# petim0/fly_bProject

Measured on AMD Instinct MI355X. Metric: env-steps/sec (PPO rollout + update), 8192 envs per GPU, higher is better.
Workload: dtype f32 (optimizer step: fp16x2 operand split; rollout policy + critic: bf16x3 operand split; fp32 accumulate)

## Files before the change

### fly_bproject_amd/csrc/fs_common.inc

```
#ifndef FS_IN
#define FS_IN 73
#endif
#ifndef FS_RING
#define FS_RING 4
#endif
typedef short s16x4 __attribute__((ext_vector_type(4)));
constexpr int FS_PX = 96, FS_P1 = 256, FS_P2 = 128, FS_P4 = 32;
template <int PITCH>
__device__ __forceinline__ int fs_key(int r)
{
    if (PITCH % 128 == 0) return ((r & 3) << 2) | ((r >> 2) & 3);
    return (r >> 2) & 3;
}
template <int PITCH>
__device__ __forceinline__ int fs_off(int r, int c) { return r * PITCH + ((((c >> 3) ^ fs_key<PITCH>(r))) << 3) + (c & 7); }
template <int PITCH> constexpr int fs_plane() { return BM * PITCH; }

__device__ __forceinline__ void fs_mfma_v(f32x16& acc, const bf16x8& a, const bf16x8& b)
{
    asm volatile("v_mfma_f32_32x32x16_bf16 %0, %1, %2, %0" : "+v"(acc) : "v"(a), "v"(b));
}
__device__ __forceinline__ void fs_mfma_v0(f32x16& acc, const bf16x8& a, const bf16x8& b)
{
    asm volatile("v_mfma_f32_32x32x16_bf16 %0, %1, %2, 0" : "=&v"(acc) : "v"(a), "v"(b));
}
__device__ __forceinline__ void fs_mfma_vg(f32x16& acc, const bf16x8& a, const bf16x8& b)
{
    asm volatile("s_nop 3\n\tv_mfma_f32_32x32x16_bf16 %0, %1, %2, %0" : "+v"(acc) : "v"(a), "v"(b));
}
__device__ __forceinline__ void fs_mfma_vg0(f32x16& acc, const bf16x8& a, const bf16x8& b)
{
    asm volatile("s_nop 3\n\tv_mfma_f32_32x32x16_bf16 %0, %1, %2, 0" : "=&v"(acc) : "v"(a), "v"(b));
}
__device__ __forceinline__ void fs_mfma_settle(f32x16& acc) { asm volatile("s_nop 7\n\ts_nop 7\n\ts_nop 3" : "+v"(acc)); }
__device__ __forceinline__ void fs_mfma_settle(f32x16& a, f32x16& b) { asm volatile("s_nop 7\n\ts_nop 7\n\ts_nop 3" : "+v"(a), "+v"(b)); }

template <int K, int PITCH, bool SWAP, bool ZERO = true, int HEAD = B3_HEAD>
__device__ __forceinline__ void fs_gemm(const WeightHeadT<HEAD>& head, const u16* __restrict__ Wb, int tile0, const u16* act, int k0,
                                        f32x16& hi, f32x16& lo, int lane)
{
    constexpr int K16 = K / 16;
    constexpr int RING = K16 < FS_RING ? K16 : FS_RING;
    constexpr int ARING = K16 < B3_ARING ? K16 : B3_ARING;
    const int r = lane & 31;
    const int key = fs_key<PITCH>(r);
    const int sh = (k0 >> 3) + (lane >> 5);
    const u16* arow = act + r * PITCH;
    const u16* bp = Wb + (long)tile0 * K16 * 1536 + lane * 8;
    Frag3 b[RING], a[ARING];
    auto aload = [&](Frag3& f, int kb) {
        const u16* q = arow + (((sh + 2 * kb) ^ key) << 3);
#pragma unroll
        for (int p = 0; p < 3; ++p) f.p[p] = *reinterpret_cast<const float4*>(q + p * fs_plane<PITCH>());
    };
#pragma unroll
    for (int s = 0; s < RING; ++s) {
        if (s < ARING) aload(a[s], s);
#pragma unroll
        for (int p = 0; p < 3; ++p)
            b[s].p[p] = s < HEAD ? head.b[s].p[p] : *reinterpret_cast<const float4*>(bp + s * 1536 + p * 512);
    }
#pragma unroll
    for (int kb = 0; kb < K16; ++kb) {
        const int s = kb % RING, sa = kb % ARING;
        __builtin_amdgcn_sched_barrier(0);
        const bf16x8 w0 = as_bf16x8(b[s].p[0]), w1 = as_bf16x8(b[s].p[1]), w2 = as_bf16x8(b[s].p[2]);
        const bf16x8 x0 = as_bf16x8(a[sa].p[0]), x1 = as_bf16x8(a[sa].p[1]), x2 = as_bf16x8(a[sa].p[2]);
        if (ZERO && kb == 0) {
            if (!SWAP) { fs_mfma_v0(lo, w0, x2); fs_mfma_v0(hi, w0, x0); } else { fs_mfma_v0(lo, x2, w0); fs_mfma_v0(hi, x0, w0); }
        } else {
            if (!SWAP) { fs_mfma_v(lo, w0, x2); fs_mfma_v(hi, w0, x0); } else { fs_mfma_v(lo, x2, w0); fs_mfma_v(hi, x0, w0); }
        }
        if (!SWAP) { fs_mfma_v(lo, w2, x0); fs_mfma_v(lo, w1, x1); fs_mfma_v(lo, w0, x1); fs_mfma_v(lo, w1, x0); }
        else { fs_mfma_v(lo, x0, w2); fs_mfma_v(lo, x1, w1); fs_mfma_v(lo, x1, w0); fs_mfma_v(lo, x0, w1); }
        __builtin_amdgcn_sched_barrier(0);
        if (kb + RING < K16) {
#pragma unroll
            for (int p = 0; p < 3; ++p) b[s].p[p] = *reinterpret_cast<const float4*>(bp + (kb + RING) * 1536 + p * 512);
        }
        if (kb + ARING < K16) aload(a[sa], kb + ARING);
    }
    fs_mfma_settle(hi, lo);
    __builtin_amdgcn_sched_barrier(0);
}

template <int K, int PITCH, bool SWAP, bool ZERO, class E, int HOST_GAPS = 6 * (K / 16), int MODE = 0>
struct FsGemmHost {
    static constexpr bool SPLIT = MODE == 1;
    static constexpr int K16 = K / 16, GAPS = 6 * K16, HALF = K16 / 2;
    static constexpr int RING = K16 < FS_RING ? K16 : FS_RING;
    static constexpr int ARING = K16 < B3_ARING ? K16 : B3_ARING;
    static_assert(!SPLIT || K16 == 16, "the split order is written for K = 256");
    static_assert(HOST_GAPS <= GAPS && (MODE == 0 || HOST_GAPS <= 6 * HALF), "the guest must be done when the second half begins");
    static constexpr bool order_ok()
    {
        unsigned seen = 0;
        for (int i = 0; i < K16; ++i) {
            const int kb = kblock(i);
            if (kb < 0 || kb >= K16 || ((seen >> kb) & 1u)) return false;
            if (MODE == 1 && ((kb & 2) != 0) != (i >= HALF)) return false;
            seen |= 1u << kb;
        }
        return true;
    }
    Frag3 b[RING], a[ARING];
    const u16 *arow, *bp;
    int sh, key;
    f32x16 &hi, &lo;
    E& e;
    __device__ __forceinline__ FsGemmHost(f32x16& hi_, f32x16& lo_, E& e_) : hi(hi_), lo(lo_), e(e_) {}
    static constexpr int kblock(int i) { return !SPLIT ? i : (i < HALF ? 4 * (i >> 1) + (i & 1) : 4 * ((i - HALF) >> 1) + 2 + (i & 1)); }
    static_assert(order_ok(), "k-step order");
    __device__ __forceinline__ void aload(Frag3& f, int kb)
    {
        const u16* q = arow + (((sh + 2 * kb) ^ key) << 3);
#pragma unroll
        for (int p = 0; p < 3; ++p) f.p[p] = *reinterpret_cast<const float4*>(q + p * fs_plane<PITCH>());
    }
    __device__ __forceinline__ void bload(Frag3& f, int kb)
    {
#pragma unroll
        for (int p = 0; p < 3; ++p) f.p[p] = *reinterpret_cast<const float4*>(bp + kb * 1536 + p * 512);
    }
    template <int J>
    __device__ __forceinline__ void gap()
    {
        if constexpr (J < HOST_GAPS) {
            constexpr int T0 = J * E::TOTAL / HOST_GAPS, T1 = (J + 1) * E::TOTAL / HOST_GAPS;
            __builtin_amdgcn_sched_barrier(0);
            run<T0, T1>();
            __builtin_amdgcn_sched_barrier(0);
        }
    }
    template <int T, int TE>
    __device__ __forceinline__ void run()
    {
        if constexpr (T < TE) { e.q(T); run<T + 1, TE>(); }
    }
    template <int I>
    __device__ __forceinline__ void steps()
    {
        if constexpr (I < K16) {
            constexpr int s = I % RING, sa = I % ARING;
            if constexpr (MODE != 0 && I == HALF) {
                if (SPLIT) __syncthreads();
#pragma unroll
                for (int u = 0; u < ARING; ++u)
                    if (HALF + u < K16) aload(a[(HALF + u) % ARING], kblock(HALF + u));
            }
            __builtin_amdgcn_sched_barrier(0);
            const bf16x8 w0 = as_bf16x8(b[s].p[0]), w1 = as_bf16x8(b[s].p[1]), w2 = as_bf16x8(b[s].p[2]);
            const bf16x8 x0 = as_bf16x8(a[sa].p[0]), x1 = as_bf16x8(a[sa].p[1]), x2 = as_bf16x8(a[sa].p[2]);
            if constexpr (ZERO && I == 0) {
                if (!SWAP) { fs_mfma_v0(lo, w0, x2); gap<0>(); fs_mfma_v0(hi, w0, x0); } else { fs_mfma_v0(lo, x2, w0); gap<0>(); fs_mfma_v0(hi, x0, w0); }
            } else {
                if (!SWAP) { fs_mfma_v(lo, w0, x2); gap<6 * I>(); fs_mfma_v(hi, w0, x0); } else { fs_mfma_v(lo, x2, w0); gap<6 * I>(); fs_mfma_v(hi, x0, w0); }
            }
            gap<6 * I + 1>();
            if (!SWAP) {
                fs_mfma_v(lo, w2, x0); gap<6 * I + 2>(); fs_mfma_v(lo, w1, x1); gap<6 * I + 3>();
                fs_mfma_v(lo, w0, x1); gap<6 * I + 4>(); fs_mfma_v(lo, w1, x0);
            } else {
                fs_mfma_v(lo, x0, w2); gap<6 * I + 2>(); fs_mfma_v(lo, x1, w1); gap<6 * I + 3>();
                fs_mfma_v(lo, x1, w0); gap<6 * I + 4>(); fs_mfma_v(lo, x0, w1);
            }
            __builtin_amdgcn_sched_barrier(0);
            if constexpr (I + RING < K16) bload(b[s], kblock(I + RING));
            if constexpr (I + ARING < K16 && !(MODE != 0 && I < HALF && I + ARING >= HALF)) aload(a[sa], kblock(I + ARING));
            gap<6 * I + 5>();
            steps<I + 1>();
        }
    }
};
template <int K, int PITCH, bool SWAP, bool ZERO = true, int HEAD = B3_HEAD, int HOST_GAPS = 6 * (K / 16), int MODE = 0, class E>
__device__ __forceinline__ void fs_gemm_host(const WeightHeadT<HEAD>& head, const u16* __restrict__ Wb, int tile0, const u16* act, int k0,
                                             f32x16& hi, f32x16& lo, int lane, E& e)
{
    typedef FsGemmHost<K, PITCH, SWAP, ZERO, E, HOST_GAPS, MODE> G;
    G g(hi, lo, e);
    const int r = lane & 31;
    g.key = fs_key<PITCH>(r);
    g.sh = (k0 >> 3) + (lane >> 5);
    g.arow = act + r * PITCH;
    g.bp = Wb + (long)tile0 * G::K16 * 1536 + lane * 8;
    static_assert(MODE != 1 || HEAD <= 2, "a head is the first k-steps IN ORDER: 0, 1 are the split order's first two as well");
#pragma unroll
    for (int s = 0; s < G::RING; ++s) {
        if (s < G::ARING && (MODE == 0 || s < G::HALF)) g.aload(g.a[s], G::kblock(s));
        if (s < HEAD) {
#pragma unroll
            for (int p = 0; p < 3; ++p) g.b[s].p[p] = head.b[s].p[p];
        } else {
            g.bload(g.b[s], G::kblock(s));
        }
    }
    g.template steps<0>();
    fs_mfma_settle(hi, lo);
    __builtin_amdgcn_sched_barrier(0);
}

template <int T, int TE, class E>
__device__ __forceinline__ void fs_run_ops(E& e)
{
    if constexpr (T < TE) { e.q(T); fs_run_ops<T + 1, TE>(e); }
}
template <int J, int GAPS, class E>
__device__ __forceinline__ void fs_host_gap(E& e)
{
    __builtin_amdgcn_sched_barrier(0);
    fs_run_ops<J * E::TOTAL / GAPS, (J + 1) * E::TOTAL / GAPS>(e);
    __builtin_amdgcn_sched_barrier(0);
}
template <int J0, int GAPS, class E>
__device__ __forceinline__ void fs_dw_host(f32x16& acc, const bf16x8 (&z)[3], const bf16x8 (&a)[3], E& e)
{
    acc = __builtin_amdgcn_mfma_f32_32x32x16_bf16(z[0], a[2], acc, 0, 0, 0); fs_host_gap<J0 + 0, GAPS>(e);
    acc = __builtin_amdgcn_mfma_f32_32x32x16_bf16(z[2], a[0], acc, 0, 0, 0); fs_host_gap<J0 + 1, GAPS>(e);
    acc = __builtin_amdgcn_mfma_f32_32x32x16_bf16(z[1], a[1], acc, 0, 0, 0); fs_host_gap<J0 + 2, GAPS>(e);
    acc = __builtin_amdgcn_mfma_f32_32x32x16_bf16(z[0], a[1], acc, 0, 0, 0); fs_host_gap<J0 + 3, GAPS>(e);
    acc = __builtin_amdgcn_mfma_f32_32x32x16_bf16(z[1], a[0], acc, 0, 0, 0); fs_host_gap<J0 + 4, GAPS>(e);
    acc = __builtin_amdgcn_mfma_f32_32x32x16_bf16(z[0], a[0], acc, 0, 0, 0); fs_host_gap<J0 + 5, GAPS>(e);
}

template <int PITCH>
__device__ __forceinline__ void fs_store4(u16* plane0, int r, int c, const float4& y)
{
    unsigned a0, b0, c0, a1, b1, c1;
    split3x2(y.x, y.y, a0, b0, c0);
    split3x2(y.z, y.w, a1, b1, c1);
    u16* q = plane0 + fs_off<PITCH>(r, c);
    *reinterpret_cast<uint2*>(q) = make_uint2(a0, a1);
    *reinterpret_cast<uint2*>(q + fs_plane<PITCH>()) = make_uint2(b0, b1);
// ... 212 lines not shown
```

### fly_bproject_amd/csrc/mlp_fused_step.inc

```
#include "fs_common.inc"
constexpr int FS_OFF_X = 0;
constexpr int FS_X_HALVES = 3 * BM * FS_PX;
constexpr int FS_OFF_H1 = FS_OFF_X + 2 * FS_X_HALVES;
constexpr int FS_OFF_H2 = FS_OFF_H1 + 3 * BM * FS_P1;
constexpr int FS_OFF_H3 = FS_OFF_H2 + 3 * BM * FS_P2;
constexpr int FS_OFF_R = FS_OFF_H3 + 3 * BM * FS_P2;
constexpr int FS_OFF_Z4 = FS_OFF_R + 4 * BM * MLP_OUT * 2;
constexpr int FS_OFF_F32 = FS_OFF_R + 3 * BM * FS_P2;
constexpr int FS_TAIL_FLOATS = MLP_H1 + MLP_H2 + MLP_H3 + MLP_OUT + 2 * BM + 2 * MLP_OUT + 4;
constexpr int FS_XS_FLOATS = BM * MLP_IN;
constexpr int FS_LDS_BYTES = FS_OFF_F32 * 2 + FS_TAIL_FLOATS * 4;
static_assert(FS_OFF_Z4 + 3 * BM * FS_P4 <= FS_OFF_F32, "split-K partials and the dZ4 planes fit region R side by side");
static_assert(FS_XS_FLOATS * 4 <= 3 * BM * FS_P2 * 2, "the staging block fits H2's region");
static_assert(FS_LDS_BYTES <= 160 * 1024, "fits one CU");

template <int PITCH, bool DUMP>
__device__ __forceinline__ void fs_epilogue_elu(const f32x16& hi, const f32x16& lo, const float* bias, int col0, u16* plane0,
                                                int lane, float* __restrict__ dump_tile, int nvalid)
{
    const int r = lane & 31;
    float4 y[4];
#pragma unroll
    for (int g = 0; g < 4; ++g) {
        const int nb = col0 + acc_n(g, lane);
// ... 486 lines not shown
        __syncthreads();
        stamp<STAMP>(stamps, 9);
        if (!STAMP) fs_split(n);
        {
            WeightHead3 wt2b;
            f32x16 cs2;
            const bool more = tile + __builtin_amdgcn_readfirstlane(grid_v) < ntiles;
            FsXStoreSlices xc(xs, Xn, tl);
#pragma unroll
            for (int t = 0; t < 2; ++t) {
                const int ct = 2 * wave + t;
                bf16x8 z1f[2][3];
                {
                    f32x16 hi, lo;
                    if (t == 0) fs_gemm<MLP_H2, FS_P2, true>(wt2, PTB + MLP_OFF_PTB2, ct, Z2, 0, hi, lo, lane);
                    else fs_gemm<MLP_H2, FS_P2, true>(wt2b, PTB + MLP_OFF_PTB2, ct, Z2, 0, hi, lo, lane);
                    if (t == 0) { stamp<STAMP>(stamps, 12); if (!STAMP) fs_split(n); }
                    if (STAMP && t == 1) stamp<STAMP>(stamps, 16);
                    if (t == 0 && more) x_fetch(tile + __builtin_amdgcn_readfirstlane(grid_v), tl);
                    bf16x8 hf[2][3], zf[2][3];
#pragma unroll
                    for (int s = 0; s < 2; ++s) fs_trws<FS_P1>(hf[s], H1, tr1, ct, s);
                    fs_trws<FS_P2>(zf[0], Z2, tr2, 0, 0);
                    unsigned q[2][3][4];
                    const fs_u32x4 hw[2][3] = {{__builtin_bit_cast(fs_u32x4, hf[0][0]), __builtin_bit_cast(fs_u32x4, hf[0][1]),
                                                __builtin_bit_cast(fs_u32x4, hf[0][2])},
                                               {__builtin_bit_cast(fs_u32x4, hf[1][0]), __builtin_bit_cast(fs_u32x4, hf[1][1]),
                                                __builtin_bit_cast(fs_u32x4, hf[1][2])}};
                    FsDz1Ops<DUMP> ez(hi, lo, hw, q, DUMP ? dump.dz1 + row0 * MLP_H1 + ct * 1024 : nullptr, lane, nvalid);
#define FS_P8_STEP(C_)                                                                                                            \
                    {                                                                                                             \
                        constexpr int c = (C_), s = c >> 2, nt = c & 3;                                                           \
                        if (c + 1 < 8) fs_trws<FS_P2>(zf[(c + 1) & 1], Z2, tr2, (c + 1) & 3, (c + 1) >> 2);                        \
                        __builtin_amdgcn_sched_barrier(0);                                                                        \
                        fs_dw_host<6 * c, 48>(aW2[nt][t], zf[c & 1], hf[s], ez);                                                  \
                        if (STAMP && t == 0 && c == 3) stamp<STAMP>(stamps, 18);                                                  \
                        if (t == 0 && nt == wave) {                           \
                            if (s == 0) fs_colsum_step<true>(cs2, zf[c & 1]); else fs_colsum_step<false>(cs2, zf[c & 1]);         \
                        }                                                                                                         \
                        __builtin_amdgcn_sched_barrier(0);                                                                        \
                    }
                    FS_P8_STEP(0) FS_P8_STEP(1) FS_P8_STEP(2) FS_P8_STEP(3) FS_P8_STEP(4) FS_P8_STEP(5) FS_P8_STEP(6) FS_P8_STEP(7)
#undef FS_P8_STEP
                    if (STAMP && t == 0) stamp<STAMP>(stamps, 17);
                    bs1[t] += ez.zsum;
#pragma unroll
                    for (int s = 0; s < 2; ++s)
#pragma unroll
                        for (int p = 0; p < 3; ++p) {
                            const fs_u32x4 qq = {q[s][p][0], q[s][p][1], q[s][p][2], q[s][p][3]};
                            z1f[s][p] = __builtin_bit_cast(bf16x8, qq);
                        }
                }
                if (t == 0) {
                    bs2 += fs_colsum_done(cs2);
                    fs_dma_drain();
                    gemm_prefetch_b3<MLP_H2>(wt2b, PTB + MLP_OFF_PTB2, 2 * wave + 1, lane);
                }
                stamp<STAMP>(stamps, t == 0 ? 13 : 15);
                if (!STAMP) fs_split(n);
                {
                    bf16x8 af[2][2][3];
                    fs_trns<FS_PX>(af[0][0], Xc, trx, 0, 0);
                    fs_trns<FS_PX>(af[0][1], Xc, trx, 0, 1);
#pragma unroll
                    for (int kt = 0; kt < 3; ++kt) {
                        if (kt + 1 < 3) {
                            fs_trns<FS_PX>(af[(kt + 1) & 1][0], Xc, trx, kt + 1, 0);
                            fs_trns<FS_PX>(af[(kt + 1) & 1][1], Xc, trx, kt + 1, 1);
                        }
                        __builtin_amdgcn_sched_barrier(0);
                        fs_dw_fill3(aW1[t][kt], z1f[0], af[kt & 1][0], xc, 18 * t + 6 * kt);
                        fs_dw_fill3(aW1[t][kt], z1f[1], af[kt & 1][1], xc, 18 * t + 6 * kt + 3);
                        __builtin_amdgcn_sched_barrier(0);
                    }
                }
                if (t == 0) stamp<STAMP>(stamps, 14);
            }
        }
        stamp<STAMP>(stamps, 10);
        if (!STAMP) fs_split(n);
        __syncthreads();
        stamp<STAMP>(stamps, 11);
        if (!STAMP) fs_split(n);
    }
    if (STAMP) stamps = reinterpret_cast<unsigned long long*>(dump.out) + ((long)blockIdx.x * 64 + 63) * FS_STAMP_SLOTS;
    stamp<STAMP>(stamps, 0);
    if (!STAMP) fs_split(n);

    const int lane = tid & 63;
    const unsigned G = gridDim.x, wg = blockIdx.x;
    constexpr unsigned S1 = fs_pad256(FS_STRIDE1), S2 = fs_pad256(FS_STRIDE2), S3 = fs_pad256(FS_STRIDE3);
    const unsigned o1 = 0, o2 = G * S1, o3 = G * (S1 + S2), o4 = G * (S1 + S2 + S3);
#pragma unroll
    for (int t = 0; t < 2; ++t)
#pragma unroll
        for (int kt = 0; kt < 3; ++kt) fs_store_tile(ws, o1, G, wg, MLP_IN_PAD, 2 * wave + t, kt, aW1[t][kt], lane);
#pragma unroll
    for (int nt = 0; nt < 4; ++nt)
#pragma unroll
        for (int t = 0; t < 2; ++t) fs_store_tile(ws, o2, G, wg, MLP_H1, nt, 2 * wave + t, aW2[nt][t], lane);
#pragma unroll
    for (int a = 0; a < 2; ++a)
#pragma unroll
        for (int b = 0; b < 2; ++b) fs_store_tile(ws, o3, G, wg, MLP_H2, 2 * (wave >> 1) + a, 2 * (wave & 1) + b, aW3[a][b], lane);
    fs_store_tile(ws, o4, G, wg, MLP_H3, 0, wave, aW4, lane);
    if (lane < 32) {
        ws[fs_slab(o2, G, wg, MLP_H2 * MLP_H1 + 32 * wave + lane)] = bs2;
        ws[fs_slab(o3, G, wg, MLP_H3 * MLP_H2 + 32 * wave + lane)] = bs3;
        if (wave == 0) ws[fs_slab(o4, G, wg, MLP_OUT * MLP_H3 + lane)] = bs4;
    }
#pragma unroll
    for (int t = 0; t < 2; ++t) {
        const float v = bs1[t] + __shfl_xor(bs1[t], 32, 64);
        if (lane < 32) ws[fs_slab(o1, G, wg, MLP_H1 * MLP_IN_PAD + 32 * (2 * wave + t) + lane)] = v;
    }
    if (STAMP) {
        asm volatile("s_waitcnt vmcnt(0)" ::: "memory");
        stamp<STAMP>(stamps, 1);
        if (!STAMP) fs_split(n);
        if (threadIdx.x == 0) stamps[2] = realtime_cu();
    }
}

constexpr int FR_OFF_X = 0;
constexpr int FR_OFF_H1 = FR_OFF_X + FS_X_HALVES;
constexpr int FR_OFF_H2 = FR_OFF_H1 + 3 * BM * FS_P1;
constexpr int FR_OFF_H3 = FR_OFF_H2 + 3 * BM * FS_P2;
constexpr int FR_OFF_PART = FR_OFF_H3 + 3 * BM * FS_P2;
constexpr int FR_OFF_F32 = FR_OFF_PART + 4 * BM * MLP_OUT * 2;
constexpr int FR_TAIL_FLOATS = MLP_H1 + MLP_H2 + MLP_H3 + MLP_OUT + 3 * 32 + BM * MLP_NACT + 4;
constexpr int FR_LDS_BYTES = FR_OFF_F32 * 2 + FR_TAIL_FLOATS * 4;
static_assert(BM * MLP_IN * 4 <= 3 * BM * FS_P2 * 2, "the observation block fits H2's region");

struct FrLds {
    u16 *X, *H1, *H2, *H3;
    float *part, *bias1, *bias2, *bias3, *bias4, *sd, *lg, *varcur, *acts, *hld, *obs;
    __device__ __forceinline__ explicit FrLds(u16* lds)
        : X(lds + FR_OFF_X), H1(lds + FR_OFF_H1), H2(lds + FR_OFF_H2), H3(lds + FR_OFF_H3),
          part(reinterpret_cast<float*>(lds + FR_OFF_PART)), bias1(reinterpret_cast<float*>(lds + FR_OFF_F32)), bias2(bias1 + MLP_H1),
          bias3(bias2 + MLP_H2), bias4(bias3 + MLP_H3), sd(bias4 + MLP_OUT), lg(sd + 32), varcur(lg + 32), acts(varcur + 32),
          hld(acts + BM * MLP_NACT), obs(reinterpret_cast<float*>(lds + FR_OFF_H2)) {}
};

__device__ __forceinline__ void policy_tile_fs_setup(const FrLds& L, const float* __restrict__ P)
{
    const int tid = threadIdx.x;
    L.bias1[tid] = P[MLP_OFF_B1 + tid];
    if (tid < MLP_H2) L.bias2[tid] = P[MLP_OFF_B2 + tid];
    else L.bias3[tid - MLP_H2] = P[MLP_OFF_B3 + tid - MLP_H2];
    if (tid < MLP_OUT) L.bias4[tid] = P[MLP_OFF_B4 + tid];
}

__device__ __forceinline__ void policy_tile_fs_head(WeightHeadT<2>& w1, const u16* __restrict__ PB)
{
    const int wave = __builtin_amdgcn_readfirstlane(threadIdx.x >> 6);
    gemm_prefetch_b3<MLP_IN_PAD>(w1, PB + MLP_OFF_PB1, 2 * wave, threadIdx.x & 63);
}
template <bool STAMP = false, bool NORM = false>
__device__ __forceinline__ void policy_tile_fs(const FrLds& L, const long tile, const u16* __restrict__ PB, const float* __restrict__ x,
                                               const long n, float* __restrict__ v_out, const float* __restrict__ smp_eps,
                                               float* __restrict__ smp_act, float* __restrict__ smp_logp, const WeightHeadT<2>& w1,
                                               unsigned long long* stamps = nullptr, const float* norm_tab = nullptr)
{
    const int tid = threadIdx.x, wave = __builtin_amdgcn_readfirstlane(tid >> 6);
    int tl = tid;
    asm volatile("" : "+v"(tl));
    const int lane = tl & 63, r = lane & 31;
    const long row0 = tile * BM;
    const int nvalid = (int)(n - row0 < BM ? n - row0 : BM);
    const int lrow = tl >> 3, lq = tl & 7;
    const bool lin = lrow < nvalid;
    float eps_pre[4];
#pragma unroll
    for (int j = 0; j < 4; ++j)
        eps_pre[j] = (lin && 4 * lq + j < MLP_NACT) ? (smp_eps + row0 * MLP_NACT)[lrow * MLP_NACT + 4 * lq + j] : 0.0f;
    if (x != nullptr) {
        const long total = n * MLP_IN, base = tile * (BM * MLP_IN) + 584L * wave;
        for (int i = lane; i < 584; i += 64) L.obs[584 * wave + i] = base + i < total ? x[base + i] : 0.0f;
    }
    static_assert(BM * MLP_IN == 4 * 584, "eight rows per wave");
    if (tid < 32) {
        const float v = tid < MLP_NACT ? L.varcur[tid] : 1.0f;
        const float s = sqrtf(v);
        L.sd[tid] = s;
        float lg = tid < MLP_NACT ? logf(s) : 0.0f;
        L.lg[tid] = lg;
#pragma unroll
        for (int o = 1; o < 32; o <<= 1) lg += __shfl_xor(lg, o, 32);
        if (tid == 0) L.hld[0] = lg;
    }
    if (NORM) {
        float* row = L.obs + (tl >> 3) * FS_IN;
        const int c0 = 12 * (tl & 7);
#pragma unroll
        for (int j = 0; j < 12; ++j)
            if (c0 + j < FS_IN) row[c0 + j] = obs_norm_apply(row[c0 + j], norm_tab[c0 + j], norm_tab[FS_IN + c0 + j], norm_tab[2 * FS_IN]);
    }
    { FsXStoreSlices xc(L.obs, L.X, tl); xc.all(); }
    __syncthreads();
    stamp<STAMP>(stamps, 1);
    WeightHeadT<2> w4;
    {
        f32x16 hi, lo;
        WeightHeadT<2> w1b, w2a;
        fs_gemm<MLP_IN_PAD, FS_PX, false>(w1, PB + MLP_OFF_PB1, 2 * wave, L.X, 0, hi, lo, lane);
        gemm_prefetch_b3<MLP_IN_PAD>(w1b, PB + MLP_OFF_PB1, 2 * wave + 1, lane);
        fs_epilogue_elu<FS_P1, false>(hi, lo, L.bias1, 64 * wave, L.H1, lane, nullptr, nvalid);
        fs_gemm<MLP_IN_PAD, FS_PX, false>(w1b, PB + MLP_OFF_PB1, 2 * wave + 1, L.X, 0, hi, lo, lane);
        gemm_prefetch_b3<MLP_H2>(w2a, PB + MLP_OFF_PB2, wave, lane);
        fs_epilogue_elu<FS_P1, false>(hi, lo, L.bias1, 64 * wave + 32, L.H1, lane, nullptr, nvalid);
        __syncthreads();
        stamp<STAMP>(stamps, 2);
        WeightHeadT<2> w2b, w3;
        gemm_prefetch_b3<MLP_H2>(w2b, PB + MLP_OFF_PB2 + 3 * MLP_H2 * (MLP_H1 / 2), wave, lane);
        fs_gemm<MLP_H2, FS_P1, false>(w2a, PB + MLP_OFF_PB2, wave, L.H1, 0, hi, lo, lane);
        fs_gemm<MLP_H2, FS_P1, false, false>(w2b, PB + MLP_OFF_PB2 + 3 * MLP_H2 * (MLP_H1 / 2), wave, L.H1, MLP_H1 / 2, hi, lo, lane);
        gemm_prefetch_b3<MLP_H2>(w3, PB + MLP_OFF_PB3, wave, lane);
        fs_epilogue_elu<FS_P2, false>(hi, lo, L.bias2, 32 * wave, L.H2, lane, nullptr, nvalid);
        __syncthreads();
        stamp<STAMP>(stamps, 3);
        gemm_prefetch_b3<32>(w4, PB + MLP_OFF_PB4 + (long)(2 * wave) * 1536, 0, lane);
        fs_gemm<MLP_H2, FS_P2, false>(w3, PB + MLP_OFF_PB3, wave, L.H2, 0, hi, lo, lane);
        fs_epilogue_elu<FS_P2, false>(hi, lo, L.bias3, 32 * wave, L.H3, lane, nullptr, nvalid);
        __syncthreads();
        stamp<STAMP>(stamps, 4);
    }
    {
        f32x16 hi, lo;
        fs_gemm<32, FS_P2, false>(w4, PB + MLP_OFF_PB4 + (long)(2 * wave) * 1536, 0, L.H3, 32 * wave, hi, lo, lane);
        float* pw = L.part + wave * (BM * MLP_OUT);
#pragma unroll
        for (int g = 0; g < 4; ++g)
            *reinterpret_cast<float4*>(pw + r * MLP_OUT + 4 * ((acc_n(g, lane) >> 2) ^ ((r >> 1) & 7))) =
                make_float4(hi[4 * g] + lo[4 * g], hi[4 * g + 1] + lo[4 * g + 1], hi[4 * g + 2] + lo[4 * g + 2],
                            hi[4 * g + 3] + lo[4 * g + 3]);
    }
    __syncthreads();
    stamp<STAMP>(stamps, 5);
    {
        const int c0 = 4 * lq;
        const int cs = 4 * (lq ^ ((lrow >> 1) & 7));
        const float4 p0 = *reinterpret_cast<const float4*>(L.part + lrow * MLP_OUT + cs);
        const float4 p1 = *reinterpret_cast<const float4*>(L.part + BM * MLP_OUT + lrow * MLP_OUT + cs);
        const float4 p2 = *reinterpret_cast<const float4*>(L.part + 2 * BM * MLP_OUT + lrow * MLP_OUT + cs);
        const float4 p3 = *reinterpret_cast<const float4*>(L.part + 3 * BM * MLP_OUT + lrow * MLP_OUT + cs);
        const float4 b4 = *reinterpret_cast<const float4*>(L.bias4 + c0);
        const float4 s4 = *reinterpret_cast<const float4*>(L.sd + c0);
        const float hld = L.hld[0];
        const float zz[4] = {(((p0.x + p1.x) + p2.x) + p3.x) + b4.x, (((p0.y + p1.y) + p2.y) + p3.y) + b4.y,
                             (((p0.z + p1.z) + p2.z) + p3.z) + b4.z, (((p0.w + p1.w) + p2.w) + p3.w) + b4.w};
        const float sdv[4] = {s4.x, s4.y, s4.z, s4.w};
        float a[4], xsq[4], yv[4];
#pragma unroll
        for (int j = 0; j < 4; ++j) {
            const int col = c0 + j;
            const float y = (col < MLP_NACT) ? elu(zz[j]) : ((col == MLP_NACT) ? zz[j] : 0.0f);
            yv[j] = y;
            a[j] = 0.0f; xsq[j] = 0.0f;
            if (col < MLP_NACT && lin) {
                a[j] = y + sdv[j] * eps_pre[j];
                const float xj = (a[j] - y) / sdv[j];
                xsq[j] = xj * xj;
            }
        }
        const float M = fs_sum8((xsq[0] + xsq[1]) + (xsq[2] + xsq[3]));
        if (lin) {
            if (v_out && lq == MLP_NACT / 4) (v_out + row0)[lrow] = yv[MLP_NACT % 4];
#pragma unroll
            for (int j = 0; j < 4; ++j)
                if (c0 + j < MLP_NACT) {
                    const float ac = fminf(fmaxf(a[j], -1.0f), 1.0f);
                    (smp_act + row0 * MLP_NACT)[lrow * MLP_NACT + c0 + j] = ac;
                    L.acts[lrow * MLP_NACT + c0 + j] = ac;
                }
            if (lq == 0) (smp_logp + row0)[lrow] = gauss_logp(M, hld);
        }
    }
    __syncthreads();
}
```

### fly_bproject_amd/csrc/mlp_mfma.hip

```cpp
#include <hip/hip_runtime.h>
#include <stdint.h>
#include <type_traits>
#include <cstdio>
#include <cstdlib>
#include "flyhip.h"
#include "mlp_layout.h"
#include "obs_norm.h"
#include "domain_rand.h"
#include "launch.h"

namespace {

#include "loss_head.inc"
#include "mlp_gemm.inc"
#include "fs_stamp.inc"
#include "mlp_forward.inc"
#include "mlp_backward.inc"
#include "mlp_grad_w.inc"
#include "mlp_fused_step.inc"
#include "mlp_adam.inc"
#include "fly_body.inc"

constexpr int RS_LDS_FLOATS = FWD_LDS_FLOATS > ENVS_PER_BLOCK * FLY_NUM_OBS ? FWD_LDS_FLOATS : ENVS_PER_BLOCK * FLY_NUM_OBS;
constexpr int RS_B3_LDS_FLOATS = FWD_B3_LDS_FLOATS > ENVS_PER_BLOCK * FLY_NUM_OBS ? FWD_B3_LDS_FLOATS : ENVS_PER_BLOCK * FLY_NUM_OBS;
static_assert(ENVS_PER_BLOCK == BM && BLOCK == THREADS, "one forward tile = one env block");
constexpr int NORM_LDS_FLOATS = OBS_NORM_TABLE + 1;
static_assert(MLP_IN == OBS_NORM_COLS && OBS_NORM_TABLE <= THREADS, "one table entry per thread");

template <bool B3, bool NORM = false, bool DR = false>
__global__ __launch_bounds__(THREADS, B3 ? 1 : 2) void rollout_step_kernel(
    const FlyConfig* __restrict__ c, FlyBuffers b, const float* __restrict__ P, const void* __restrict__ PF,
    const float* __restrict__ x, long n, const float* __restrict__ eps, const float* __restrict__ var, int var_steps,
    float var_decay, float var_min, float* __restrict__ act, float* __restrict__ logp, float* __restrict__ v_out,
    const int* __restrict__ var_base)
{
    constexpr int ARENA = B3 ? RS_B3_LDS_FLOATS : RS_LDS_FLOATS;
    __shared__ __attribute__((aligned(16))) float lds[ARENA + (NORM ? NORM_LDS_FLOATS : 0)];
    float* const norm_tab = NORM ? lds + ARENA : nullptr;
    if (NORM) obs_norm_load(norm_tab, c);
    var_steps -= var_base ? *var_base : 0;
    constexpr int PH_ALL = PH_SCALE | PH_RESET | PH_INTEGRATE | PH_OBS | PH_PROGRESS | PH_REWARD;
    FlyRegs st;
    fly_load<PH_ALL, DR>(st, c, b, blockIdx.x);
    if (NORM) __syncthreads();
    if (B3)
        forward_body_b3<false, false, NORM>(lds, blockIdx.x, 1L << 40, P, static_cast<const u16*>(PF), x, n, nullptr, v_out, nullptr,
                                            nullptr, nullptr, nullptr, eps, var, act, logp, nullptr, var_steps, var_decay, var_min,
                                            nullptr, nullptr, false, norm_tab);
    else
        forward_body<false, false, NORM>(lds, blockIdx.x, 1L << 40, P, static_cast<const float*>(PF), x, n, nullptr, v_out, nullptr,
                                         nullptr, nullptr, nullptr, eps, var, act, logp, nullptr, var_steps, var_decay, var_min,
                                         norm_tab);
    __builtin_amdgcn_fence(__ATOMIC_RELEASE, "workgroup");
    __builtin_amdgcn_s_waitcnt(0);
    __syncthreads();
    fly_body<PH_ALL, DR>(c, act, b, lds, blockIdx.x, st);
}

__device__ __forceinline__ void store_pose(float* __restrict__ poses, int t, const FlyRegs& nx)
{
    const int sub = threadIdx.x;
    if (sub >= LANES_PER_ENV) return;
    float* p = poses + (long)t * FLY_POSE_FLOATS;
    if (sub < FLY_NUM_LEGS) {
#pragma unroll
        for (int i = 0; i < 3; ++i) p[7 + 3 * sub + i] = nx.jq[i];
    }
    if (sub == LANES_PER_ENV - 1) {
        p[0] = nx.r.px; p[1] = nx.r.py; p[2] = nx.r.pz; p[3] = nx.r.qx; p[4] = nx.r.qy; p[5] = nx.r.qz; p[6] = nx.r.qw;
    }
}

template <bool B3, int WPS, bool REC, bool NORM = false, bool DR = false>
__global__ __launch_bounds__(THREADS, WPS) void rollout_all_kernel(
    const FlyConfig* __restrict__ c, FlyBuffers b, const float* __restrict__ P, const void* __restrict__ PF,
    float* __restrict__ obs_ring, long n, const float* __restrict__ eps_all, const float* __restrict__ var, float var_decay,
    float var_min, float* __restrict__ act_all, float* __restrict__ logp_all, float* __restrict__ v_ring,
    float* __restrict__ reward_all, int T, const int* __restrict__ rows_applied, int64_t* __restrict__ reset_rows,
    int64_t* __restrict__ progress_rows, float* __restrict__ poses)
{
    constexpr int ARENA = B3 ? RS_B3_LDS_FLOATS : RS_LDS_FLOATS;
    __shared__ __attribute__((aligned(16))) float lds[ARENA + 32 + BM * MLP_NACT + (NORM ? NORM_LDS_FLOATS : 0)];
    float* const norm_tab = NORM ? lds + ARENA + 32 + BM * MLP_NACT : nullptr;
    if (NORM) obs_norm_load(norm_tab, c);
    constexpr int PH_ALL = PH_SCALE | PH_RESET | PH_INTEGRATE | PH_OBS | PH_PROGRESS | PH_REWARD;
    float* varcur = lds + ARENA;
    float* acts = B3 ? lds + ARENA + 32 : nullptr;
    if (threadIdx.x < MLP_NACT) varcur[threadIdx.x] = var[threadIdx.x];
    FlyRegs st;
    fly_load<PH_ALL, DR>(st, c, b, blockIdx.x);
    __syncthreads();
    const bool whole = (long)(blockIdx.x + 1) * BM <= n;
    for (int t = 0; t < T; ++t) {
        const float* x = obs_ring + (long)t * n * FLY_NUM_OBS;
        float* act = act_all + (long)t * n * MLP_NACT;
        b.obs = obs_ring + (long)(t + 1) * n * FLY_NUM_OBS;
        b.reward = reward_all + (long)t * n;
        if (reset_rows) { b.reset = reset_rows + (long)t * n; b.progress = progress_rows + (long)t * n; }
        const bool in_lds = B3 && whole;
        if (B3)
            forward_body_b3<false, false, NORM>(lds, blockIdx.x, 1L << 40, P, static_cast<const u16*>(PF), x, n, nullptr,
                                                v_ring + (long)t * n, nullptr, nullptr, nullptr, nullptr, eps_all + (long)t * n * MLP_NACT,
                                                varcur, act, logp_all + (long)t * n, nullptr, 0, var_decay, var_min,
                                                in_lds && t > 0 ? lds : nullptr, in_lds ? acts : nullptr, t > 0, norm_tab);
        else
            forward_body<false, false, NORM>(lds, blockIdx.x, 1L << 40, P, static_cast<const float*>(PF), x, n, nullptr,
                                             v_ring + (long)t * n, nullptr, nullptr, nullptr, nullptr, eps_all + (long)t * n * MLP_NACT,
                                             varcur, act, logp_all + (long)t * n, nullptr, 0, var_decay, var_min, norm_tab);
        if (!in_lds) {
            __builtin_amdgcn_fence(__ATOMIC_RELEASE, "workgroup");
            __builtin_amdgcn_s_waitcnt(0);
        }
        __syncthreads();
        FlyRegs nx;
        fly_body<PH_ALL, DR>(c, act, b, lds, blockIdx.x, st, &nx, in_lds ? acts : nullptr);
        if (REC && blockIdx.x == 0) store_pose(poses, t, nx);
        st = nx;
        if (threadIdx.x < MLP_NACT && var_decay > 0.0f) varcur[threadIdx.x] = fmaxf(var_min, varcur[threadIdx.x] - var_decay);
        if (!in_lds) asm volatile("s_waitcnt vmcnt(0)" ::: "memory");
        __syncthreads();
    }
}

template <bool STAMP, bool MULTI, bool REC, bool NORM = false, bool DR = false>
__global__ __launch_bounds__(THREADS, 1) void rollout_all_fs_kernel(
    const FlyConfig* __restrict__ c, FlyBuffers b, const float* __restrict__ P, const u16* __restrict__ PB,
    float* __restrict__ obs_ring, long n, const float* __restrict__ eps_all, const float* __restrict__ var, float var_decay,
    float var_min, float* __restrict__ act_all, float* __restrict__ logp_all, float* __restrict__ v_ring,
    float* __restrict__ reward_all, int T, int64_t* __restrict__ reset_rows, int64_t* __restrict__ progress_rows,
    void* __restrict__ aux)
{
    static_assert(!(STAMP && REC) && !(STAMP && NORM) && !(STAMP && DR), "the stamped diagnostic form neither records, normalises nor randomises");
    unsigned long long* const stamps = static_cast<unsigned long long*>(aux);
    float* const poses = static_cast<float*>(aux);
    extern __shared__ __attribute__((aligned(16))) u16 fr_lds[];
    const FrLds L(fr_lds);
    constexpr int PH_ALL = PH_SCALE | PH_RESET | PH_INTEGRATE | PH_OBS | PH_PROGRESS | PH_REWARD;
    policy_tile_fs_setup(L, P);
    float* const norm_tab = NORM ? reinterpret_cast<float*>(fr_lds) + FR_LDS_BYTES / 4 : nullptr;
    if (NORM) obs_norm_load(norm_tab, c);
    int64_t* const reset0 = b.reset;
    int64_t* const progress0 = b.progress;
    const long ntiles = n / BM;
    long tile = blockIdx.x;
    do {
        unsigned long long* st_tile = STAMP ? stamps + tile * (T + 1) * 8 : nullptr;
        if (threadIdx.x < 32) L.varcur[threadIdx.x] = threadIdx.x < MLP_NACT ? var[threadIdx.x] : 1.0f;
        b.reset = reset0; b.progress = progress0;
        FlyRegs st;
        fly_load<PH_ALL, DR>(st, c, b, (int)tile);
        WeightHeadT<2> w1;
        policy_tile_fs_head(w1, PB);
        __syncthreads();
        if (STAMP && threadIdx.x == 0) st_tile[6] = realtime_cu();
        for (int t = 0; t < T; ++t) {
            stamp<STAMP>(st_tile, 8 * t);
            float* act = act_all + (long)t * n * MLP_NACT;
            b.obs = obs_ring + (long)(t + 1) * n * FLY_NUM_OBS;
            b.reward = reward_all + (long)t * n;
            if (reset_rows) { b.reset = reset_rows + (long)t * n; b.progress = progress_rows + (long)t * n; }
            policy_tile_fs<STAMP, NORM>(L, tile, PB, t == 0 ? obs_ring : nullptr, n, v_ring + (long)t * n, eps_all + (long)t * n * MLP_NACT,
                                        act, logp_all + (long)t * n, w1, STAMP ? st_tile + 8 * t : nullptr, norm_tab);
            stamp<STAMP>(st_tile, 8 * t + 7);
            policy_tile_fs_head(w1, PB);
            FlyRegs nx;
            fly_body<PH_ALL, DR>(c, act, b, L.obs, (int)tile, st, &nx, L.acts);
            if (REC && tile == 0) store_pose(poses, t, nx);
            st = nx;
            if (threadIdx.x < MLP_NACT && var_decay > 0.0f) L.varcur[threadIdx.x] = fmaxf(var_min, L.varcur[threadIdx.x] - var_decay);
            __syncthreads();
        }
        stamp<STAMP>(st_tile, 8 * T);
        if (STAMP && threadIdx.x == 0) st_tile[8 * T + 1] = realtime_cu();
        tile += gridDim.x;
    } while (MULTI && tile < ntiles);
}

}

extern "C" hipError_t flyhip_launch_rollout_all(const FlyConfig* dcfg, const FlyBuffers* b, const float* P, const float* PF,
                                                float* obs_ring, int64_t n, const float* eps_all, const float* var,
                                                float var_decay, float var_min, float* act_all, float* logp_all, float* v_ring,
                                                float* reward_all, int T, const int* rows_applied, const uint16_t* PB,
                                                int64_t* reset_rows, int64_t* progress_rows, void* stream,
                                                unsigned long long* stamps, float* poses, int norm, int dr)
{
    const dim3 grid((unsigned)((n + BM - 1) / BM));
    const int cus = device_cus();
    const bool one_per_cu = (int)grid.x <= cus;
    const char* fs_env = getenv("FLY_ROLLOUT_FS");
    const bool fs_off = fs_env != nullptr && fs_env[0] == '0';
    if (stamps && (poses || norm || dr)) return hipErrorInvalidValue;
    const bool rec = poses != nullptr;
    if (PB && n % BM == 0 && !fs_off) {
        const dim3 grid_fs(one_per_cu ? grid.x : (unsigned)cus);
        static_assert(FR_LDS_BYTES % 4 == 0, "the table follows the image");
        auto fs = [&](void* aux, auto S, auto M, auto R, auto N, auto D) {
            return launch_kernel<rollout_all_fs_kernel<S.value, M.value, R.value, N.value, D.value>>(
                grid_fs, THREADS, FR_LDS_BYTES + (N.value ? NORM_LDS_FLOATS * 4 : 0), stream, dcfg, *b, P, PB, obs_ring, (long)n, eps_all,
                var, var_decay, var_min, act_all, logp_all, v_ring, reward_all, T, reset_rows, progress_rows, aux);
        };
        constexpr std::false_type no{};
        const bool multi = !one_per_cu;
        if (stamps) return with_bools([&](auto M) { return fs(stamps, std::true_type{}, M, no, no, no); }, multi);
        return with_bools([&](auto M, auto R, auto N, auto D) { return fs(poses, no, M, R, N, D); }, multi, rec, norm != 0, dr != 0);
    }
    if (stamps) return hipErrorInvalidValue;
    auto ra = [&](auto B3, auto WPS, const void* pf) {
        return with_bools([&](auto R, auto N, auto D) {
            return launch_kernel<rollout_all_kernel<B3.value, WPS.value, R.value, N.value, D.value>>(
                grid, THREADS, 0, stream, dcfg, *b, P, pf, obs_ring, (long)n, eps_all, var, var_decay, var_min, act_all, logp_all, v_ring,
                reward_all, T, rows_applied, reset_rows, progress_rows, poses);
        }, rec, norm != 0, dr != 0);
    };
    if (PB) return ra(std::true_type{}, int_c<1>{}, PB);
    return one_per_cu ? ra(std::false_type{}, int_c<1>{}, PF) : ra(std::false_type{}, int_c<2>{}, PF);
}

extern "C" hipError_t flyhip_launch_mlp_forward(const float* P, const float* PF, const float* x, int64_t n, float* mu_out,
                                                float* v_out, float* out_save, float* h1_save, float* h2_save,
                                                float* h3_save, const uint16_t* PB, void* stream)
{
    if (PB) {
        const long tiles = (n + BM - 1) / BM;
        const int grid = (int)tiles;
        hipLaunchKernelGGL(mlp_forward_b3_kernel, dim3(grid), dim3(THREADS), 0, (hipStream_t)stream, P, PB, x, (long)n, mu_out,
                           v_out, out_save, h1_save, h2_save, h3_save, (const float*)nullptr, (const float*)nullptr,
                           (float*)nullptr, (float*)nullptr, 0, 0.0f, 0.0f, (const int*)nullptr);
        return hipGetLastError();
    }
    const long tiles = (n + BM - 1) / BM;
    const int grid = (int)(tiles <= 4 * PERSIST_GRID ? tiles : PERSIST_GRID);
    hipLaunchKernelGGL(mlp_forward_kernel<false>, dim3(grid), dim3(THREADS), 0, (hipStream_t)stream, P, PF, x, (long)n,
                       mu_out, v_out, out_save, h1_save, h2_save, h3_save, (const float*)nullptr, (const float*)nullptr,
                       (float*)nullptr, (float*)nullptr, (unsigned long long*)nullptr, 0, 0.0f, 0.0f, (const int*)nullptr);
    return hipGetLastError();
}

extern "C" hipError_t flyhip_launch_mlp_forward_sample(const float* P, const float* PF, const float* x, int64_t n,
                                                       const float* eps, const float* var, int var_steps,
                                                       float var_decay, float var_min, float* act_out,
                                                       float* logp_out, float* mu_out, float* v_out, const uint16_t* PB,
                                                       const int* var_base, void* stream)
{
    if (PB) {
        const long tiles = (n + BM - 1) / BM;
        const int grid = (int)tiles;
        hipLaunchKernelGGL(mlp_forward_b3_kernel, dim3(grid), dim3(THREADS), 0, (hipStream_t)stream, P, PB, x, (long)n, mu_out,
                           v_out, (float*)nullptr, (float*)nullptr, (float*)nullptr, (float*)nullptr, eps, var, act_out,
                           logp_out, var_steps, var_decay, var_min, var_base);
        return hipGetLastError();
    }
    const long tiles = (n + BM - 1) / BM;
    const int grid = (int)(tiles <= 4 * PERSIST_GRID ? tiles : PERSIST_GRID);
    hipLaunchKernelGGL(mlp_forward_kernel<false>, dim3(grid), dim3(THREADS), 0, (hipStream_t)stream, P, PF, x, (long)n,
                       mu_out, v_out, (float*)nullptr, (float*)nullptr, (float*)nullptr, (float*)nullptr, eps,
                       var, act_out, logp_out, (unsigned long long*)nullptr, var_steps, var_decay, var_min, var_base);
    return hipGetLastError();
}

extern "C" int flyhip_debug_mlp_forward_stamped(const float* P, const float* PF, const float* x, int64_t n,
                                                float* out_save, float* h1_save, float* h2_save, float* h3_save,
                                                unsigned long long* stamps, void* stream, int grid_override)
{
    const long tiles = (n + BM - 1) / BM;
    const int grid = grid_override > 0 ? grid_override : (int)(tiles <= 4 * PERSIST_GRID ? tiles : PERSIST_GRID);
    hipLaunchKernelGGL(mlp_forward_kernel<true>, dim3(grid), dim3(THREADS), 0, (hipStream_t)stream, P, PF, x, (long)n,
                       (float*)nullptr, (float*)nullptr, out_save, h1_save, h2_save, h3_save, (const float*)nullptr,
                       (const float*)nullptr, (float*)nullptr, (float*)nullptr, stamps, 0, 0.0f, 0.0f, (const int*)nullptr);
    return (int)hipGetLastError();
}

extern "C" hipError_t flyhip_launch_mlp_backward_dx(const float* PT, const float* out_saved, const float* h1,
                                                    const float* h2, const float* h3, const float* action,
                                                    const float* old_logp, const float* adv, const float* target,
                                                    const float* var, int64_t n, float inv_batch, float clip,
                                                    float* dz4, float* dz3, float* dz2, float* dz1, float* loss_part,
                                                    const uint16_t* PTB, void* stream)
{
    if (PTB) {
        hipLaunchKernelGGL(mlp_backward_dx_b3_kernel, dim3((unsigned)((n + BM - 1) / BM)), dim3(THREADS), 0, (hipStream_t)stream,
                           PTB, out_saved, h1, h2, h3, action, old_logp, adv, target, var, (long)n, inv_batch, clip, dz4, dz3,
                           dz2, dz1, loss_part);
        return hipGetLastError();
    }
    const int grid = (int)((n + BM - 1) / BM);
    hipLaunchKernelGGL(mlp_backward_dx_kernel, dim3(grid), dim3(THREADS), 0, (hipStream_t)stream, PT, out_saved,
                       h1, h2, h3, action, old_logp, adv, target, var, (long)n, inv_batch, clip, dz4, dz3, dz2, dz1,
                       loss_part);
    return hipGetLastError();
}

static int kGradWgs[4] = {80, 100, 52, 24};
static int kGradWgsB3[4] = {72, 88, 64, 32};
static bool gw_env_read = false;
static void gw_read_env()
{
    if (gw_env_read) return;
    gw_env_read = true;
    const char* e = getenv("FLYHIP_GW_SPLIT");
    int v[4];
    if (e && sscanf(e, "%d,%d,%d,%d", &v[0], &v[1], &v[2], &v[3]) == 4 && v[0] > 0 && v[1] > 0 && v[2] > 0 && v[3] > 0 &&
        v[0] + v[1] + v[2] + v[3] <= 1024)
        for (int i = 0; i < 4; ++i) kGradWgs[i] = kGradWgsB3[i] = v[i];
}

static int g_fb_consumer_shift = 0;
extern "C" void flyhip_debug_set_fwd_bwd_consumer_shift(int shift) { g_fb_consumer_shift = shift; }

extern "C" hipError_t flyhip_launch_mlp_fwd_bwd(const float* P, const float* PF, const float* PT, const float* x, int64_t n,
                                                float* out_save, float* h1_save, float* h2_save, float* h3_save,
                                                const float* action, const float* old_logp, const float* adv,
                                                const float* target, const float* var, float inv_batch, float clip,
                                                float* dz4, float* dz3, float* dz2, float* dz1, float* loss_part,
                                                int* flags, int epoch, int* err, const uint16_t* PB, const uint16_t* PTB,
                                                int coherent, void* stream)
{
// ... 167 lines not shown
```

Before: 68.63 million.

## Keep layer-1 and layer-3 policy weights resident in AGPRs across rollout steps

New measurement: 68.91 million, median of 2. About the same (+0.4%).

```diff
diff --git a/fly_bproject_amd/csrc/fs_common.inc b/fly_bproject_amd/csrc/fs_common.inc
--- a/fly_bproject_amd/csrc/fs_common.inc
+++ b/fly_bproject_amd/csrc/fs_common.inc
@@ -78,6 +78,62 @@
 #pragma unroll
             for (int p = 0; p < 3; ++p) b[s].p[p] = *reinterpret_cast<const float4*>(bp + (kb + RING) * 1536 + p * 512);
         }
+        if (kb + ARING < K16) aload(a[sa], kb + ARING);
+    }
+    fs_mfma_settle(hi, lo);
+    __builtin_amdgcn_sched_barrier(0);
+}
+
+struct FragR { bf16x8 p[3]; };
+__device__ __forceinline__ void fs_mfma_a(f32x16& acc, const bf16x8& a, const bf16x8& b)
+{
+    asm volatile("v_mfma_f32_32x32x16_bf16 %0, %1, %2, %0" : "+v"(acc) : "a"(a), "v"(b));
+}
+__device__ __forceinline__ void fs_mfma_a0(f32x16& acc, const bf16x8& a, const bf16x8& b)
+{
+    asm volatile("v_mfma_f32_32x32x16_bf16 %0, %1, %2, 0" : "=&v"(acc) : "a"(a), "v"(b));
+}
+template <int K16, int W0, int N, int M>
+__device__ __forceinline__ void fs_resident_load(FragR (&w)[M], const u16* __restrict__ Wb, int tile0, int lane)
+{
+    static_assert(W0 + N <= M && N <= K16, "fragment range");
+    const u16* bp = Wb + (long)tile0 * K16 * 1536 + lane * 8;
+#pragma unroll
+    for (int s = 0; s < N; ++s)
+#pragma unroll
+        for (int p = 0; p < 3; ++p) {
+            w[W0 + s].p[p] = as_bf16x8(*reinterpret_cast<const float4*>(bp + s * 1536 + p * 512));
+            asm volatile("" : "+a"(w[W0 + s].p[p]));
+        }
+}
+template <int K, int PITCH, bool ZERO, int W0, int M>
+__device__ __forceinline__ void fs_gemm_res(const FragR (&w)[M], const u16* act, int k0, f32x16& hi, f32x16& lo, int lane)
+{
+    constexpr int K16 = K / 16;
+    constexpr int ARING = K16 < B3_ARING ? K16 : B3_ARING;
+    static_assert(W0 + K16 <= M, "fragment range");
+    const int r = lane & 31;
+    const int key = fs_key<PITCH>(r);
+    const int sh = (k0 >> 3) + (lane >> 5);
+    const u16* arow = act + r * PITCH;
+    Frag3 a[ARING];
+    auto aload = [&](Frag3& f, int kb) {
+        const u16* q = arow + (((sh + 2 * kb) ^ key) << 3);
+#pragma unroll
+        for (int p = 0; p < 3; ++p) f.p[p] = *reinterpret_cast<const float4*>(q + p * fs_plane<PITCH>());
+    };
+#pragma unroll
+    for (int s = 0; s < ARING; ++s) aload(a[s], s);
+#pragma unroll
+    for (int kb = 0; kb < K16; ++kb) {
+        const int sa = kb % ARING;
+        __builtin_amdgcn_sched_barrier(0);
+        const bf16x8 &w0 = w[W0 + kb].p[0], &w1 = w[W0 + kb].p[1], &w2 = w[W0 + kb].p[2];
+        const bf16x8 x0 = as_bf16x8(a[sa].p[0]), x1 = as_bf16x8(a[sa].p[1]), x2 = as_bf16x8(a[sa].p[2]);
+        if (ZERO && kb == 0) { fs_mfma_a0(lo, w0, x2); fs_mfma_a0(hi, w0, x0); }
+        else { fs_mfma_a(lo, w0, x2); fs_mfma_a(hi, w0, x0); }
+        fs_mfma_a(lo, w2, x0); fs_mfma_a(lo, w1, x1); fs_mfma_a(lo, w0, x1); fs_mfma_a(lo, w1, x0);
+        __builtin_amdgcn_sched_barrier(0);
         if (kb + ARING < K16) aload(a[sa], kb + ARING);
     }
     fs_mfma_settle(hi, lo);
diff --git a/fly_bproject_amd/csrc/mlp_fused_step.inc b/fly_bproject_amd/csrc/mlp_fused_step.inc
--- a/fly_bproject_amd/csrc/mlp_fused_step.inc
+++ b/fly_bproject_amd/csrc/mlp_fused_step.inc
@@ -662,16 +662,22 @@
     if (tid < MLP_OUT) L.bias4[tid] = P[MLP_OFF_B4 + tid];
 }
 
-__device__ __forceinline__ void policy_tile_fs_head(WeightHeadT<2>& w1, const u16* __restrict__ PB)
+
+struct FrResident { FragR w1[10], w3[8]; };
+__device__ __forceinline__ void policy_tile_fs_resident(FrResident& R, const u16* __restrict__ PB)
 {
-    const int wave = __builtin_amdgcn_readfirstlane(threadIdx.x >> 6);
-    gemm_prefetch_b3<MLP_IN_PAD>(w1, PB + MLP_OFF_PB1, 2 * wave, threadIdx.x & 63);
+    const int wave = __builtin_amdgcn_readfirstlane(threadIdx.x >> 6), lane = threadIdx.x & 63;
+    fs_resident_load<MLP_IN_PAD / 16, 0, 5>(R.w1, PB + MLP_OFF_PB1, 2 * wave, lane);
+    fs_resident_load<MLP_IN_PAD / 16, 5, 5>(R.w1, PB + MLP_OFF_PB1, 2 * wave + 1, lane);
+    fs_resident_load<MLP_H2 / 16, 0, 8>(R.w3, PB + MLP_OFF_PB3, wave, lane);
 }
+
 template <bool STAMP = false, bool NORM = false>
 __device__ __forceinline__ void policy_tile_fs(const FrLds& L, const long tile, const u16* __restrict__ PB, const float* __restrict__ x,
                                                const long n, float* __restrict__ v_out, const float* __restrict__ smp_eps,
-                                               float* __restrict__ smp_act, float* __restrict__ smp_logp, const WeightHeadT<2>& w1,
-                                               unsigned long long* stamps = nullptr, const float* norm_tab = nullptr)
+                                               float* __restrict__ smp_act, float* __restrict__ smp_logp,
+                                               const FrResident& R, unsigned long long* stamps = nullptr,
+                                               const float* norm_tab = nullptr)
 {
     const int tid = threadIdx.x, wave = __builtin_amdgcn_readfirstlane(tid >> 6);
     int tl = tid;
@@ -713,27 +719,26 @@
     WeightHeadT<2> w4;
     {
         f32x16 hi, lo;
-        WeightHeadT<2> w1b, w2a;
-        fs_gemm<MLP_IN_PAD, FS_PX, false>(w1, PB + MLP_OFF_PB1, 2 * wave, L.X, 0, hi, lo, lane);
-        gemm_prefetch_b3<MLP_IN_PAD>(w1b, PB + MLP_OFF_PB1, 2 * wave + 1, lane);
+        WeightHeadT<2> w2a;
+        gemm_prefetch_b3<MLP_H2>(w2a, PB + MLP_OFF_PB2, wave, lane);
+        fs_gemm_res<MLP_IN_PAD, FS_PX, true, 0>(R.w1, L.X, 0, hi, lo, lane);
         fs_epilogue_elu<FS_P1, false>(hi, lo, L.bias1, 64 * wave, L.H1, lane, nullptr, nvalid);
-        fs_gemm<MLP_IN_PAD, FS_PX, false>(w1b, PB + MLP_OFF_PB1, 2 * wave + 1, L.X, 0, hi, lo, lane);
-        gemm_prefetch_b3<MLP_H2>(w2a, PB + MLP_OFF_PB2, wave, lane);
+        fs_gemm_res<MLP_IN_PAD, FS_PX, true, 5>(R.w1, L.X, 0, hi, lo, lane);
         fs_epilogue_elu<FS_P1, false>(hi, lo, L.bias1, 64 * wave + 32, L.H1, lane, nullptr, nvalid);
         __syncthreads();
         stamp<STAMP>(stamps, 2);
-        WeightHeadT<2> w2b, w3;
+        WeightHeadT<2> w2b;
         gemm_prefetch_b3<MLP_H2>(w2b, PB + MLP_OFF_PB2 + 3 * MLP_H2 * (MLP_H1 / 2), wave, lane);
         fs_gemm<MLP_H2, FS_P1, false>(w2a, PB + MLP_OFF_PB2, wave, L.H1, 0, hi, lo, lane);
         fs_gemm<MLP_H2, FS_P1, false, false>(w2b, PB + MLP_OFF_PB2 + 3 * MLP_H2 * (MLP_H1 / 2), wave, L.H1, MLP_H1 / 2, hi, lo, lane);
-        gemm_prefetch_b3<MLP_H2>(w3, PB + MLP_OFF_PB3, wave, lane);
+        gemm_prefetch_b3<32>(w4, PB + MLP_OFF_PB4 + (long)(2 * wave) * 1536, 0, lane);
         fs_epilogue_elu<FS_P2, false>(hi, lo, L.bias2, 32 * wave, L.H2, lane, nullptr, nvalid);
         __syncthreads();
         stamp<STAMP>(stamps, 3);
-        gemm_prefetch_b3<32>(w4, PB + MLP_OFF_PB4 + (long)(2 * wave) * 1536, 0, lane);
-        fs_gemm<MLP_H2, FS_P2, false>(w3, PB + MLP_OFF_PB3, wave, L.H2, 0, hi, lo, lane);
+        fs_gemm_res<MLP_H2, FS_P2, true, 0>(R.w3, L.H2, 0, hi, lo, lane);
         fs_epilogue_elu<FS_P2, false>(hi, lo, L.bias3, 32 * wave, L.H3, lane, nullptr, nvalid);
-        __syncthreads();
+        asm volatile("s_waitcnt lgkmcnt(0)" ::: "memory");
+        __builtin_amdgcn_wave_barrier();
         stamp<STAMP>(stamps, 4);
     }
     {
diff --git a/fly_bproject_amd/csrc/mlp_mfma.hip b/fly_bproject_amd/csrc/mlp_mfma.hip
--- a/fly_bproject_amd/csrc/mlp_mfma.hip
+++ b/fly_bproject_amd/csrc/mlp_mfma.hip
@@ -142,6 +142,8 @@
     int64_t* const reset0 = b.reset;
     int64_t* const progress0 = b.progress;
     const long ntiles = n / BM;
+    FrResident R;
+    policy_tile_fs_resident(R, PB);
     long tile = blockIdx.x;
     do {
         unsigned long long* st_tile = STAMP ? stamps + tile * (T + 1) * 8 : nullptr;
@@ -149,8 +151,6 @@
         b.reset = reset0; b.progress = progress0;
         FlyRegs st;
         fly_load<PH_ALL, DR>(st, c, b, (int)tile);
-        WeightHeadT<2> w1;
-        policy_tile_fs_head(w1, PB);
         __syncthreads();
         if (STAMP && threadIdx.x == 0) st_tile[6] = realtime_cu();
         for (int t = 0; t < T; ++t) {
@@ -160,9 +160,8 @@
             b.reward = reward_all + (long)t * n;
             if (reset_rows) { b.reset = reset_rows + (long)t * n; b.progress = progress_rows + (long)t * n; }
             policy_tile_fs<STAMP, NORM>(L, tile, PB, t == 0 ? obs_ring : nullptr, n, v_ring + (long)t * n, eps_all + (long)t * n * MLP_NACT,
-                                        act, logp_all + (long)t * n, w1, STAMP ? st_tile + 8 * t : nullptr, norm_tab);
+                                        act, logp_all + (long)t * n, R, STAMP ? st_tile + 8 * t : nullptr, norm_tab);
             stamp<STAMP>(st_tile, 8 * t + 7);
-            policy_tile_fs_head(w1, PB);
             FlyRegs nx;
             fly_body<PH_ALL, DR>(c, act, b, L.obs, (int)tile, st, &nx, L.acts);
             if (REC && tile == 0) store_pose(poses, t, nx);
```
